# orottier/web-audio-api-rs

Measured on AMD Instinct MI355X. Metric: render quanta/sec (48kHz, 128-frame), higher is better.
Workload: dtype f64

## Files before the change

### web-audio-api-rs_amd/csrc/waa_biquad_lanes.hip

```cpp
#include <hip/hip_runtime.h>

#include <algorithm>
#include <cstdlib>
#include <type_traits>

#include "waa_internal.hpp"
#include "waa_stream_common.hpp"

namespace waa {

namespace {
struct V2 {
  double x, y;
};
struct M2 {
  double a, b, c, d;
};
__device__ __forceinline__ M2 mm(const M2& x, const M2& y) {
  M2 r;
  r.a = __builtin_fma(x.a, y.a, x.b * y.c);
  r.b = __builtin_fma(x.a, y.b, x.b * y.d);
  r.c = __builtin_fma(x.c, y.a, x.d * y.c);
  r.d = __builtin_fma(x.c, y.b, x.d * y.d);
  return r;
// ... 294 lines not shown
    for (int j = 0; j < 8; j++) {
      const int r = j * 8 + (lane >> 3);
      const uint32_t sr = g * 64u + (uint32_t)r;
      const bool r_live = sr < n_streams;
      const uint32_t ri = sr / (uint32_t)d.nch, rc = sr % (uint32_t)d.nch;
      orow[j] = r_live ? (uint32_t)((uint64_t)ri * d.out.inst_stride + (uint64_t)rc * d.out.ch_stride + f_tile + (uint64_t)(lane & 7) * 4)
                       : 0xFFFFFFFFu;
      if (FAST && d.debug == 1) orow[j] = (uint32_t)(((uint64_t)tile * n_groups + g) * 64 * TILE + r * CHUNK + (lane & 7) * 4);
    }
  }
  const uint64_t f_end = (uint64_t)d.n_quanta * RQ;
  const int n_chunk = f_tile + TILE <= f_end ? NCHUNK : (int)((f_end - f_tile + CHUNK - 1) / CHUNK);
  for (int c = 0; c < n_chunk; c++) {
    if (FAST || !slow_tile)
      stage_chunk(0, raw);
    else
      stage_chunk_slow(0, c);
    stage_tab(0);
    if (c + 1 < n_chunk) {
      if (FAST)
        fetch_chunk_fast(raw);
      else if (!slow_tile)
        fetch_chunk(c + 1, raw);
      fetch_tab((c + 1 + rot) & (NCHUNK - 1));
    }
    lds_sync();
    float* row = lds + lane * ROWF;
    const double* tb = tabs;
    if (d.debug == 3) {
    } else if (PASS == 0) {
#pragma unroll
      for (int k8 = 0; k8 < CHUNK / 8; k8++) {
        const f4v va = *reinterpret_cast<const f4v*>(row + k8 * 8), vb = *reinterpret_cast<const f4v*>(row + k8 * 8 + 4);
        const float xs[8] = {va.x, va.y, va.z, va.w, vb.x, vb.y, vb.z, vb.w};
#pragma unroll
        for (int e = 0; e < 8; e++) {
          const d2v h = *reinterpret_cast<const d2v*>(tb + 2 * (k8 * 8 + e));
          const double xd = (double)xs[e];
          z1 = __builtin_fma(h.x, xd, z1);
          z2 = __builtin_fma(h.y, xd, z2);
        }
        __builtin_amdgcn_sched_barrier(0);
      }
    } else {
#pragma unroll
      for (int k4 = 0; k4 < CHUNK / 4; k4++) {
        float yo[4];
        const f4v xv = *reinterpret_cast<const f4v*>(row + k4 * 4);
        const float x4[4] = {xv.x, xv.y, xv.z, xv.w};
#pragma unroll
        for (int h = 0; h < 2; h++) {
          double cs[10];
#pragma unroll
          for (int e = 0; e < 5; e++) {
            const d2v v = *reinterpret_cast<const d2v*>(tb + k4 * 20 + h * 10 + 2 * e);
            cs[2 * e] = v.x;
            cs[2 * e + 1] = v.y;
          }
#pragma unroll
          for (int e = 0; e < 2; e++) {
            const double b0 = cs[e * 5 + 0], b1 = cs[e * 5 + 1], b2 = cs[e * 5 + 2], a1 = cs[e * 5 + 3], a2 = cs[e * 5 + 4];
            const double xd = (double)x4[h * 2 + e];
            double y = (b0 * xd + b1 * x1) + b2 * x2;
            y = (y - a1 * y1) - a2 * y2;
            if (!__builtin_isfinite(y)) y = 0.;
            x2 = x1;
            x1 = xd;
            y2 = y1;
            y1 = y;
            float o = (float)y;
            if (d.n_gain > 0 && g0 != 1.f) o *= g0;
            if (d.n_gain > 1 && g1 != 1.f) o *= g1;
            yo[h * 2 + e] = mute ? 0.f : o;
          }
          __builtin_amdgcn_sched_barrier(0);
        }
        *reinterpret_cast<f4v*>(row + k4 * 4) = f4v{yo[0], yo[1], yo[2], yo[3]};
        __builtin_amdgcn_sched_barrier(0);
      }
    }
    lds_sync();
    if (PASS == 1) {
#pragma unroll
      for (int j = 0; j < 8; j++) {
        const int r = j * 8 + (lane >> 3);
        const f4v v = *reinterpret_cast<const f4v*>(lds + r * ROWF + (lane & 7) * 4);
        if (orow[j] != 0xFFFFFFFFu) {
          __builtin_nontemporal_store(v, (WAA_GLOBAL_AS f4v*)(d.out.base + orow[j]));
          orow[j] += FAST ? row_step : (uint32_t)CHUNK;
        }
      }
      lds_sync();
    }
  }
  if (PASS == 1) {
    for (int c = n_chunk; c < NCHUNK; c++) {
#pragma unroll
      for (int j = 0; j < 8; j++)
        if (orow[j] != 0xFFFFFFFFu) {
          __builtin_nontemporal_store(f4v{0.f, 0.f, 0.f, 0.f}, (WAA_GLOBAL_AS f4v*)(d.out.base + orow[j]));
          orow[j] += FAST ? row_step : (uint32_t)CHUNK;
        }
    }
  }
  if (!live) return;
  if (PASS == 0) {
    double* zp = d.z + ((uint64_t)tile * n_streams + sid) * 2;
    zp[0] = z1;
    zp[1] = z2;
  } else if (tile + 1 == d.tile1) {
    st[0] = x1;
    st[1] = x2;
    st[2] = y1;
    st[3] = y2;
  }
}

__global__ __launch_bounds__(256) void biquad_lanes_chain_kernel(const BiquadLanesDesc d) {
  const uint32_t n_streams = d.n_inst * (uint32_t)d.nch;
  const uint32_t sid = blockIdx.x * 256 + threadIdx.x;
  if (sid >= n_streams) return;
  const uint32_t inst = sid / (uint32_t)d.nch;
  const int ch = (int)(sid % (uint32_t)d.nch);
  const double* st = d.state + (uint64_t)inst * STATE_STRIDE + ch * 4;
  double s1 = st[2], s2 = st[3];
  for (uint32_t t0 = d.tile0; t0 < d.tile1; t0 += 8) {
    double zz[8][2];
#pragma unroll
    for (int k = 0; k < 8; k++) {
      const uint32_t t = t0 + k < d.tile1 ? t0 + k : d.tile1 - 1;
      const double* zp = d.z + ((uint64_t)t * n_streams + sid) * 2;
      zz[k][0] = load_global(zp);
      zz[k][1] = load_global(zp + 1);
    }
#pragma unroll
    for (int k = 0; k < 8; k++) {
      const uint32_t t = t0 + k;
      if (t >= d.tile1) break;
      double* sp = d.sin + ((uint64_t)t * n_streams + sid) * 2;
      sp[0] = s1;
      sp[1] = s2;
      const double* pt = d.ht + (uint64_t)t * BIQUAD_HT_WORDS + 2 * TILE + 4;
      const double n1 = __builtin_fma(pt[0], s1, __builtin_fma(pt[1], s2, zz[k][0]));
      const double n2 = __builtin_fma(pt[2], s1, __builtin_fma(pt[3], s2, zz[k][1]));
      s1 = n1;
      s2 = n2;
    }
  }
  double* xs = d.z + ((uint64_t)d.tile0 * n_streams + sid) * 2;
  xs[0] = st[0];
  xs[1] = st[1];
}

void launch_biquad_tile_digest(const BiquadLanesDesc& d, void* stream) {
  hipLaunchKernelGGL(biquad_tile_digest_kernel, dim3(d.n_tiles), dim3(64), 0, (hipStream_t)stream, d);
}
void launch_biquad_lanes(const BiquadLanesDesc& d0, void* stream) {
  BiquadLanesDesc d = d0;
  d.debug = measure_switch("WAA_LANES_DEBUG") ? (uint32_t)atoi(measure_switch("WAA_LANES_DEBUG")) : 0u;
  const uint32_t n_streams = d.n_inst * (uint32_t)d.nch, n_groups = (n_streams + 63u) / 64u;
  const size_t lds_a = 64 * ROWF * sizeof(float) + CHUNK * 2 * sizeof(double);
  const size_t lds_b = 64 * ROWF * sizeof(float) + CHUNK * 5 * sizeof(double);
  const uint32_t tf = measure_switch("WAA_LANES_GENERAL") ? d.tile0 : std::min(std::max(d.fast_tiles, d.tile0), d.tile1);
  auto pass = [&](auto pass_c) {
    constexpr int PASS = decltype(pass_c)::value;
    const size_t lds = (PASS == 0 ? lds_a : lds_b) + (measure_switch("WAA_LANES_LDS_PAD") ? (size_t)atoi(measure_switch("WAA_LANES_LDS_PAD")) : 0);
    if (tf > d.tile0) {
      d.lt0 = d.tile0;
      d.lt1 = tf;
      hipLaunchKernelGGL((biquad_lanes_kernel<PASS, true>), dim3((tf - d.tile0) * n_groups), dim3(64), lds, (hipStream_t)stream, d);
    }
    if (tf < d.tile1) {
      d.lt0 = tf;
      d.lt1 = d.tile1;
      hipLaunchKernelGGL((biquad_lanes_kernel<PASS, false>), dim3((d.tile1 - tf) * n_groups), dim3(64), lds, (hipStream_t)stream, d);
    }
  };
  pass(std::integral_constant<int, 0>{});
  hipLaunchKernelGGL(biquad_lanes_chain_kernel, dim3((n_streams + 255) / 256), dim3(256), 0, (hipStream_t)stream, d);
  pass(std::integral_constant<int, 1>{});
}

}
```

### web-audio-api-rs_amd/csrc/waa_internal.hpp

```cpp
#pragma once
#include <cstdint>
#include <cstdlib>

#include "waa_conv_noise.hpp"

namespace waa {

inline const char* measure_switch(const char* name) {
#ifdef WAA_MEASURE
  return getenv(name);
#else
  (void)name;
  return nullptr;
#endif
}

void raise_lds_limit(const void* kernel);

constexpr int RQ = 128;
constexpr int TILE_K = 32;
constexpr int TILE = 64 * TILE_K;
constexpr int QUANTA_PER_TILE = TILE / RQ;
constexpr int MAX_OPS = 12;
constexpr int MAX_INPUTS = 4;
// ... 4 lines not shown
  const float* base;
  uint64_t stride;
  int32_t mode;
  int32_t pad;
};

struct SignalRef {
  float* base;
  uint64_t inst_stride;
  uint64_t ch_stride;
  int32_t nch;
  int32_t pad;
};

enum : uint32_t { Q_SILENT = 0, Q_FAST = 1, Q_SLOW = 2, Q_FAST_LOOP = 3 };
struct QRec {
  int64_t start;
  uint32_t mode;
  uint32_t pad;
};
struct SlowRec {
  int32_t prev;
  int32_t next;
  double k;
};
struct SrcSchedule {
  const QRec* qrec;
  const SlowRec* slow;
  const uint8_t* tile_fast;
};
struct SrcInst {
  const float* base;
  uint64_t ch_stride;
  uint64_t frames;
  uint32_t sched;
  uint32_t aligned;
  SrcSchedule sc;
  int64_t linear_start;
  uint32_t fast_prefix;
  uint32_t linear_all;
};

enum : int32_t { IN_SILENT = 0, IN_SIGNAL = 1, IN_SOURCE = 2, IN_CONSTANT = 3, IN_DELAYED = 4 };
struct InputRef {
  int32_t kind;
  int32_t nch;
  SignalRef sig;
  const SrcInst* src;
  const SrcSchedule* sched;
  ParamRef offset;
  const int64_t* active;
  double sample_rate;
  int32_t num_quanta;
  int32_t feedback;
  uint64_t valid;
  ParamRef gain;
  int32_t has_gain;
  uint32_t fast_tiles;
  float delay_lo, delay_hi;
};

enum : int32_t {
  OP_GAIN = 1,
  OP_BIQUAD = 2,
  OP_WAVESHAPER = 3,
  OP_STEREO_PAN = 4,
  OP_PANNER = 5,
  OP_MIX = 6,
  OP_IIR = 7,
  OP_PARAM_ADD = 8
};
struct OpDesc {
  int32_t kind;
  int32_t nch_in;
  int32_t nch_out;
  int32_t i1;
  int32_t i2;
  int32_t i0;
  ParamRef p0;
  ParamRef p1;
  ParamRef p2;
  ParamRef p3;
  ParamRef p4;
  const void* ptr0;
  void* ptr1;
  const void* ptr2;
  uint64_t u0;
};

struct ChainDesc {
  int32_t n_inputs;
  int32_t in_nch;
  int32_t in_interp;
  int32_t n_ops;
  InputRef in[MAX_INPUTS];
  OpDesc ops[MAX_OPS];
  SignalRef out;
  uint32_t n_inst;
  uint32_t n_tiles;
  uint32_t n_quanta;
  uint32_t xcd_remap;
  uint32_t tile0, tile1;
  int32_t lds_curve_op;
  int32_t tile_major;
  uint32_t persist_block;
  uint32_t pad;
};

struct BiquadStreamDesc {
  InputRef in;
  const double* coefs;
  uint64_t coef_stride;
  int32_t vary;
  int32_t pad0;
  double* state;
  const double* hp;
  ParamRef gain[2];
  int32_t n_gain;
  int32_t nch;
  SignalRef out;
  uint32_t n_inst;
  uint32_t n_tiles;
  uint32_t n_quanta;
  uint32_t dup_out;
  uint32_t tile0, tile1;
};
void launch_biquad_stream(const BiquadStreamDesc& d, void* stream);
constexpr int BIQUAD_SCAN_PW = 88;
struct BiquadScanCtl {
  uint32_t* counter;
  uint32_t counter_base[8];
  double* payload;
  const double* pw;
  uint32_t* error;
};
void launch_biquad_scan_powers(const double* coefs, uint64_t coef_stride, double* pw, uint32_t n_inst, void* stream);
void launch_biquad_scan(const BiquadStreamDesc& d, const BiquadScanCtl& ctl, uint32_t* issued, void* stream);

constexpr int BIQUAD_HT_WORDS = 2 * TILE + 8;
struct BiquadLanesDesc {
  InputRef in;
  const double* coefs;
  double* ht;
  double* z;
  double* sin;
  double* state;
  ParamRef gain[2];
  int32_t n_gain, nch;
  SignalRef out;
  uint32_t n_inst, n_tiles, n_quanta, tile0, tile1;
  uint32_t fast_tiles;
  uint32_t lt0, lt1;
  uint32_t debug, pad;
};
void launch_biquad_tile_digest(const BiquadLanesDesc& d, void* stream);
void launch_biquad_lanes(const BiquadLanesDesc& d, void* stream);

struct IirStreamDesc {
  InputRef in;
  const double* coef;
  const double* pow;
  double* state;
  int32_t ns;
  int32_t nch;
  SignalRef out;
  uint32_t n_inst;
  uint32_t n_tiles;
  uint32_t n_quanta;
  uint32_t exact;
  uint32_t tile0, tile1;
  uint32_t coef_stride, pow_stride;
};
int iir_padded_states(int n_states);
void launch_iir_stream(const IirStreamDesc& d, void* stream);

struct CompRow {
  float thr, lo, hi, half_knee;
  float knee_partial, ratio, makeup, pad;
  float a_tau, a_one, r_tau, r_one;
};
struct CompDesc {
  SignalRef in;
  uint64_t in_valid;
  SignalRef out;
  float* xl;
  const CompRow* rows;
  uint32_t row_inst_stride, row_q_stride;
  uint32_t n_inst, n_quanta;
  uint64_t frames;
  uint32_t delay_frames;
  int32_t nch;
};
void launch_compressor_level(const CompDesc& d, void* stream);
void launch_compressor_detector(const CompDesc& d, void* stream);
void launch_compressor_apply(const CompDesc& d, void* stream);

enum : int32_t { RT_CHANNEL = 0, RT_DOWN2 = 1, RT_DOWN4 = 2, RT_DOWN6 = 3 };
struct RouteTerm {
  const float* base;
  uint64_t inst_stride, ch_stride;
  int32_t mode;
  int32_t ch;
};
struct RouteDesc {
  SignalRef out;
  const RouteTerm* terms;
  const uint32_t* row_off;
  uint32_t n_inst, rows;
  uint64_t frames;
};
void launch_route(const RouteDesc& d, void* stream);

struct ConvTerm {
  int32_t in_ch, ir_ch, out_ch, pad;
};
struct Cplx {
  float re, im;
};
struct ConvDesc {
  SignalRef in, out;
  int32_t n_terms;
  int32_t cin, cout;
  int32_t n;
  int32_t block;
  int32_t parts;
  int32_t nb;
  int32_t fft3;
  ConvTerm terms[4];
  const Cplx* H;
  Cplx* X;
  Cplx* Y;
  const Cplx* tw;
  const float* ir;
  uint64_t ir_len;
  uint64_t frames;
  uint64_t in_valid;
  uint32_t n_inst, n_pairs;
  int32_t ir_nch, pad1;
  int32_t kb0, kb1;
  int32_t mac_grid_order, pad2;
  const double* pre_coefs;
  uint64_t pre_coef_stride;
  double* pre_state;
  uint64_t ir_inst_stride;
  int32_t per_inst, pad3;
};
struct AnalyserDesc {
  SignalRef sig;
  uint32_t n_inst;
  int32_t fft_size;
  uint64_t frames_written;
  float smoothing;
  float min_db, max_db;
  int32_t pad;
  const float* window;
  const Cplx* tw;
  const Cplx* tw_full;
  const float* prev;
  float* db_out;
  uint8_t* byte_out;
  float* time_out;
  const uint8_t* code;
  uint64_t code_stride;
};
void launch_analyser(const AnalyserDesc& d, void* stream);
struct AnalyserSeriesDesc {
  AnalyserDesc a;
  int32_t first, hop;
  int32_t pulls;
  int32_t run;
  int32_t stage_span;
  int32_t lin;
  uint64_t frames;
  float* db_out;
  uint8_t* byte_out;
  float* time_out;
  uint8_t* tbyte_out;
};
void analyser_series_shape(AnalyserSeriesDesc* d);
void launch_analyser_series_fft(const AnalyserSeriesDesc& d, void* stream);
void launch_analyser_series_smooth(const AnalyserSeriesDesc& d, void* stream);
void launch_analyser_series_bytes(const AnalyserSeriesDesc& d, void* stream);
void launch_analyser_series_time(const AnalyserSeriesDesc& d, void* stream);
constexpr int DIRECT_MAX_TAPS = 128;
void launch_conv_direct(const ConvDesc& d, void* stream);
void launch_conv_ir_spectra(const ConvDesc& d, void* stream);
void launch_conv_forward(const ConvDesc& d, void* stream);
void launch_conv_mac(const ConvDesc& d, void* stream);
void launch_conv_inverse(const ConvDesc& d, void* stream);
void launch_conv3_ir_spectra(const ConvDesc& d, void* stream);
void launch_conv3_forward(const ConvDesc& d, void* stream);
void launch_conv3_inverse(const ConvDesc& d, void* stream);
void launch_conv_inst_direct(const ConvDesc& d, void* stream);
void launch_conv_inst_mac(const ConvDesc& d, void* stream);

struct DelayDesc {
  SignalRef in, out;
  ParamRef delay;
  double sample_rate;
  uint64_t frames;
  int32_t num_quanta;
  int32_t nch;
  uint32_t n_inst;
  uint32_t n_quanta;
  uint32_t tile0, tile1;
  int32_t in_cycle;
  int32_t pad;
  double quantum_duration;
};
// ... 434 lines not shown
```

### web-audio-api-rs_amd/csrc/waa_plan.cpp

```cpp
#include <array>
#include <set>

#include <memory>

#include "waa_host.hpp"
#include "waa_plan_parts.hpp"

namespace waa {
namespace host {

int prepare_source_input(waa_batch* b, uint32_t id, InputRef* in);
int validate_plan(waa_batch* b);

int device_timeline_param(waa_batch* b, const ParamStore& p, ParamRef* ref) {
  if (p.dev_ready) {
    *ref = p.dev_ref;
    return 0;
  }
  std::vector<TlHeader> hdr(b->n_inst);
  std::vector<TlEvent> events;
  std::vector<float> curves;
  for (uint32_t i = 0; i < b->n_inst; i++) {
    TlHeader& h = hdr[i];
    std::memset(&h, 0, sizeof h);
// ... 566 lines not shown
    bool serial = false;
    std::string desc;
    for (auto& o : ops) {
      serial |= o.kind == OP_BIQUAD;
      char t[64];
      if (o.kind == OP_MIX)
        snprintf(t, sizeof t, "MIX(%d->%d)", o.nch_in, o.nch_out);
      else if (o.kind == OP_BIQUAD)
        snprintf(t, sizeof t, "BIQUAD(%s)", o.i0 == 0 ? "const" : o.i0 == 1 ? "k-rate" : "a-rate");
      else
        snprintf(t, sizeof t, "%s", op_name(o.kind));
      desc += desc.empty() ? t : std::string(",") + t;
    }
    std::string ins;
    for (auto& in : inputs) {
      char t[48];
      snprintf(t, sizeof t, "%s%s:%dch", in.has_gain ? "gain*" : "", input_kind_name(in.kind), in.nch);
      ins += ins.empty() ? t : std::string("+") + t;
    }
    plan_note(b, "chain %s C=%d in=[%s]->%dch ops=[%s] out=%dch", serial ? "serial" : "parallel", cmax, ins.c_str(), in_nch,
              desc.c_str(), out.nch);
  }
  return 0;
}

int temp_signal(waa_batch* b, int nch, SignalRef* out) {
  float* p = nullptr;
  int e = dev_alloc(b, &p, (size_t)b->n_inst * nch * b->lp);
  if (e) return e;
  *out = SignalRef{p, (uint64_t)nch * b->lp, b->lp, nch, 0};
  return 0;
}

int emit_segments(waa_batch* b, std::vector<InputRef> inputs, int in_nch, int in_interp, const std::vector<OpDesc>& ops,
                  const SignalRef& out) {
  bool any_stream = false;
  const int max_mode = measure_switch("WAA_NO_KRATE_STREAM") ? 0 : (measure_switch("WAA_NO_ARATE_STREAM") ? 1 : 2);
  auto streams = [&](const OpDesc& o) { return o.kind == OP_IIR || (o.kind == OP_BIQUAD && o.i0 <= max_mode && o.nch_in <= MAX_CH); };
  for (auto& o : ops) any_stream |= streams(o);
  if (!any_stream) return push_chain_step(b, inputs, in_nch, in_interp, ops, out);
  std::vector<OpDesc> pending;
  int cur_nch = in_nch;
  size_t i = 0;
  while (i < ops.size()) {
    const OpDesc& o = ops[i];
    if (!streams(o)) {
      pending.push_back(o);
      cur_nch = o.nch_out;
      i++;
      continue;
    }
    const bool iir_exact = o.kind == OP_IIR && o.i0 < 0;
    const bool plain = pending.empty() && inputs.size() == 1 && !inputs[0].has_gain &&
                       ((inputs[0].kind == IN_SOURCE && !iir_exact) || (inputs[0].kind == IN_SIGNAL && inputs[0].valid == 0)) &&
                       inputs[0].nch == cur_nch;
    if (!plain) {
      SignalRef tmp;
      int e = temp_signal(b, cur_nch, &tmp);
      if (e) return e;
      if ((e = push_chain_step(b, inputs, in_nch, in_interp, pending, tmp))) return e;
      pending.clear();
      InputRef in{};
      in.kind = IN_SIGNAL;
      in.nch = cur_nch;
      in.sig = tmp;
      inputs.assign(1, in);
      in_nch = cur_nch;
    }
    size_t j = i + 1;
    if (o.kind == OP_BIQUAD)
      while (j < ops.size() && j - i <= 2 && ops[j].kind == OP_GAIN && ops[j].p0.mode == 0 && ops[j].nch_in == cur_nch) j++;
    const bool dup = o.kind == OP_BIQUAD && o.i0 == 0 && cur_nch == 1 && out.nch == 2 && j + 1 == ops.size() && ops[j].kind == OP_MIX &&
                     ops[j].nch_in == 1 && ops[j].nch_out == 2 && ops[j].i0 == WAA_INTERP_SPEAKERS && !measure_switch("WAA_NO_STREAM_DUP");
    SignalRef seg_out = out;
    if (!dup && (j < ops.size() || out.nch != cur_nch)) {
      int e = temp_signal(b, cur_nch, &seg_out);
      if (e) return e;
    }
    if (o.kind == OP_IIR) {
      Step st;
      st.kind = StepKind::IirStream;
      IirStreamDesc& q = st.iir;
      std::memset(&q, 0, sizeof q);
      q.in = inputs[0];
      q.coef = reinterpret_cast<const double*>(o.ptr0);
      q.pow = reinterpret_cast<const double*>(o.ptr2);
      q.state = reinterpret_cast<double*>(o.ptr1);
      q.ns = std::abs(o.i0);
      q.coef_stride = (uint32_t)o.u0;
      q.pow_stride = o.u0 && !iir_exact ? 6u * (uint32_t)(q.ns * q.ns) : 0u;
      q.exact = 0u;
      if (iir_exact) {
        const double streams = (double)b->n_inst * cur_nch;
        const double lane_cost = std::ceil(streams / 64. / 1024.) * (12. * q.ns + 32.);
        const double row_cost = std::ceil(streams / 4. / 1024.) * 64.;
        q.exact = (row_cost < lane_cost && !measure_switch("WAA_IIR_LANE")) || measure_switch("WAA_IIR_ROW") ? 2u : 1u;
      }
      q.nch = cur_nch;
      q.out = seg_out;
      q.n_inst = b->n_inst;
      q.n_tiles = b->n_tiles;
      q.tile0 = 0;
      q.tile1 = b->n_tiles;
      q.n_quanta = b->n_quanta;
      char name[40], per[40] = "";
      snprintf(name, sizeof name, "%s<%d%s>", q.exact == 2 ? "iir_row_kernel" : q.exact == 1 ? "iir_lane_kernel" : "iir_stream_kernel", q.ns,
               q.coef_stride ? ",inst" : "");
      st.profile_slot = slot_for(b, name);
      b->steps.push_back(st);
      if (q.coef_stride) snprintf(per, sizeof per, " coef=per-instance(%d)", o.i1);
      plan_note(b, "%s states=%d in=%s:%dch out=%s%s", q.exact == 2 ? "iir_exact(row)" : q.exact == 1 ? "iir_exact(lane)" : "iir_stream", q.ns,
                input_kind_name(inputs[0].kind), cur_nch, seg_out.base == out.base ? "final" : "temp", per);
      InputRef in{};
      in.kind = IN_SIGNAL;
      in.nch = cur_nch;
      in.sig = seg_out;
      inputs.assign(1, in);
      in_nch = cur_nch;
      i = j;
      if (i == ops.size() && seg_out.base == out.base) return 0;
      continue;
    }
    if (o.kind == OP_BIQUAD && o.i0 == 2 && !dup && b->steps[(size_t)o.i1].coef.rows == 1 && !measure_switch("WAA_ARATE_STREAM") &&
        (inputs[0].kind == IN_SIGNAL || inputs[0].kind == IN_SOURCE) &&
        (uint64_t)b->n_inst * seg_out.inst_stride < (1ull << 32)) {
      Step& cstep = b->steps[(size_t)o.i1];
      Step& dstep = b->steps[(size_t)o.i1 + 1];
      cstep.coef.lane_major = 0;
      const size_t n_streams = (size_t)b->n_inst * cur_nch;
      double *ht = nullptr, *z = nullptr, *sin = nullptr;
      int e;
      if ((e = dev_alloc(b, &ht, (size_t)b->n_tiles * BIQUAD_HT_WORDS)) || (e = dev_alloc(b, &z, (size_t)b->n_tiles * n_streams * 2)) ||
          (e = dev_alloc(b, &sin, (size_t)b->n_tiles * n_streams * 2)))
        return e;
      BiquadLanesDesc L;
      std::memset(&L, 0, sizeof L);
      L.in = inputs[0];
      L.coefs = cstep.coef.coefs;
      L.ht = ht;
      L.z = z;
      L.sin = sin;
      L.state = reinterpret_cast<double*>(o.ptr1);
      L.n_gain = (int)(j - i - 1);
      for (size_t k = i + 1; k < j; k++) L.gain[k - i - 1] = ops[k].p0;
      L.nch = cur_nch;
      L.out = seg_out;
      L.n_inst = b->n_inst;
      L.n_tiles = b->n_tiles;
      L.n_quanta = b->n_quanta;
      L.tile0 = 0;
      L.tile1 = b->n_tiles;
      L.fast_tiles = inputs[0].kind == IN_SOURCE ? inputs[0].fast_tiles
                                                 : (inputs[0].valid ? (uint32_t)std::min<uint64_t>(inputs[0].valid / TILE, b->n_tiles) : b->n_tiles);
      dstep.kind = StepKind::BiquadTileDigest;
      dstep.lanes = L;
      dstep.profile_slot = slot_for(b, "biquad_tile_digest_kernel");
      Step ls;
      ls.kind = StepKind::BiquadLanes;
      ls.lanes = L;
      ls.profile_slot = slot_for(b, "biquad_lanes_kernel");
      b->steps.push_back(ls);
      plan_note(b, "biquad_lanes(a-rate, shared table: one lane per stream, tiles in parallel) in=%s:%dch gains=%d out=%s",
                input_kind_name(inputs[0].kind), cur_nch, L.n_gain, seg_out.base == out.base ? "final" : "temp");
      InputRef in{};
      in.kind = IN_SIGNAL;
      in.nch = cur_nch;
      in.sig = seg_out;
      inputs.assign(1, in);
      in_nch = cur_nch;
      i = j;
      if (i == ops.size() && seg_out.base == out.base) return 0;
      continue;
    }
    Step st;
    st.kind = StepKind::BiquadStream;
    BiquadStreamDesc& q = st.bq;
    std::memset(&q, 0, sizeof q);
    q.in = inputs[0];
    q.coefs = reinterpret_cast<const double*>(o.ptr0);
    q.coef_stride = o.u0;
    q.vary = o.i0;
    if (o.i0 == 2) {
      Step& cstep = b->steps[(size_t)o.i1];
      cstep.coef.lane_major = 1;
      if (cstep.coef.rows == 1 && !measure_switch("WAA_NO_ARATE_DIGEST")) {
        Step& hstep = b->steps[(size_t)o.i1 + 1];
        double* dhp = nullptr;
        int e = dev_alloc(b, &dhp, (size_t)b->n_tiles * HP_WORDS * 64);
        if (e) return e;
        hstep.hp.coefs = cstep.coef.coefs;
        hstep.hp.hp = dhp;
        hstep.hp.n_tiles = b->n_tiles;
        q.hp = dhp;
        q.vary = 3;
      }
    }
    q.state = reinterpret_cast<double*>(o.ptr1);
    q.n_gain = (int)(j - i - 1);
    for (size_t k = i + 1; k < j; k++) q.gain[k - i - 1] = ops[k].p0;
    q.nch = cur_nch;
    q.out = seg_out;
    q.dup_out = dup ? 1u : 0u;
    q.n_inst = b->n_inst;
    q.n_tiles = b->n_tiles;
    q.tile0 = 0;
    q.tile1 = b->n_tiles;
    q.n_quanta = b->n_quanta;
    st.profile_slot = slot_for(b, "biquad_stream_kernel");
    if (q.vary == 0 && !b->dry && measure_switch("WAA_BIQUAD_SCAN")) {
      const size_t n_streams = (size_t)b->n_inst * cur_nch;
      if (!b->scan_counter) {
        int e = dev_alloc(b, &b->scan_counter, 8 * 16 + 16);
        if (e) return e;
        b->state_bufs.push_back({b->scan_counter, (8 * 16 + 16) * sizeof(uint32_t)});
      }
      double *payload = nullptr, *pw = nullptr;
      int e;
      if ((e = dev_alloc(b, &payload, n_streams * b->n_tiles * 8)) || (e = dev_alloc(b, &pw, (size_t)b->n_inst * BIQUAD_SCAN_PW)))
        return e;
      b->ones_bufs.push_back({payload, n_streams * b->n_tiles * 8 * sizeof(double)});
      launch_biquad_scan_powers(q.coefs, q.coef_stride, pw, b->n_inst, b->stream);
      HIP_TRY(hipGetLastError());
      st.scan.counter = b->scan_counter;
      st.scan.error = b->scan_counter + 8 * 16;
      st.scan.payload = payload;
      st.scan.pw = pw;
      st.profile_slot = slot_for(b, "biquad_scan_kernel");
    }
    b->steps.push_back(st);
    if (dup) {
      plan_note(b, "biquad_stream in=%s:1ch gains=%d out=final (both channels: the speakers up-mix 1 -> 2 behind it)",
                input_kind_name(inputs[0].kind), q.n_gain);
      return 0;
    }
    plan_note(b, "biquad_stream%s in=%s:%dch gains=%d out=%s",
              q.vary == 3 ? "(a-rate, shared table)" : q.vary == 2 ? "(a-rate, per-instance table)" : q.vary ? "(k-rate)" : "",
              input_kind_name(inputs[0].kind),
              cur_nch, q.n_gain, seg_out.base == out.base ? "final" : "temp");
    InputRef in{};
    in.kind = IN_SIGNAL;
    in.nch = cur_nch;
    in.sig = seg_out;
    inputs.assign(1, in);
    in_nch = cur_nch;
    i = j;
    if (i == ops.size() && seg_out.base == out.base) return 0;
  }
  return push_chain_step(b, inputs, in_nch, in_interp, pending, out);
}

bool is_delay(const waa_batch* b, uint32_t id) { return b->nodes[id].desc.kind == WAA_NODE_DELAY; }
void vertex_targets(const waa_batch* b, uint32_t v, const std::vector<uint8_t>& cut, std::vector<uint32_t>& out) {
  const uint32_t id = v & ~VTX_READER;
  if (!(v & VTX_READER) && is_delay(b, id)) {
    if (!cut[id]) out.push_back(id | VTX_READER);
    return;
  }
  for (auto& e : b->edges) {
    if (e.from != id) continue;
    out.push_back(is_delay(b, e.to) && (e.to_input & 0x80000000u) ? (e.to | VTX_READER) : e.to);
  }
}

int materialise_automation(waa_batch* b) {
  const double sample_rate = (double)b->sr, dt = 1. / sample_rate;
  for (Node& n : b->nodes)
    for (size_t pk = 0; pk < n.params.size(); pk++) {
      ParamStore& p = n.params[pk];
      if (p.timelines.empty()) continue;
      bool shared = p.timelines_shared && p.timelines[0];
      for (uint32_t i = 1; i < b->n_inst && shared; i++) shared = p.cst[i] == p.cst[0] && p.timelines[i];
      {
        const uint32_t kind = n.desc.kind;
        const bool consumable = kind == WAA_NODE_GAIN || kind == WAA_NODE_BIQUAD || kind == WAA_NODE_DELAY ||
                                kind == WAA_NODE_STEREO_PANNER || kind == WAA_NODE_CONSTANT_SOURCE ||
                                kind == WAA_NODE_OSCILLATOR ||
                                (kind == WAA_NODE_PANNER && pk >= 6 && n.desc.i[0] != WAA_PANNING_HRTF);
        const bool want = measure_switch("WAA_DEVICE_AUTOMATION") ? true : !shared;
        bool arrivals = false;
        for (const auto& tl : p.timelines) arrivals |= tl && tl->has_arrivals();
        if (consumable && !p.k_rate && want && !arrivals && !b->dry && !measure_switch("WAA_HOST_AUTOMATION")) {
          p.dev_tl = true;
          continue;
        }
      }
      for (uint32_t inst = 0; inst < (shared ? 1u : b->n_inst); inst++) {
        Timeline* tl = p.timelines[inst].get();
        if (!tl) continue;
        float buf[RQ];
        ParamBlock run;
        run.inst = shared ? WAA_ALL_INSTANCES : inst;
        run.nq = 0;
        auto flush = [&] {
          if (run.nq) p.blocks.push_back(run);
          run.nq = 0;
          run.v.clear();
        };
        for (uint32_t q = 0; q < b->n_quanta; q++) {
          const double block_time = (double)((uint64_t)q * RQ) / sample_rate;
          if (int ea = tl->apply_arrivals(q)) return ea;
          const uint32_t len = tl->compute(block_time, dt, RQ, buf);
          if (run.nq && run.vpq != len) flush();
          if (!run.nq) {
            run.q0 = q;
            run.vpq = len;
          }
// ... 1284 lines not shown
```

### web-audio-api-rs_amd/csrc/waa_plan_check.cpp

```cpp
#include <array>
#include <set>

#include "waa_host.hpp"
#include "waa_plan_parts.hpp"

namespace waa {
namespace host {

void io_param(const ParamRef& p, StepIo& io) {
  if (p.base && p.mode == 2) io.reads.push_back(p.base);
}
void io_input(const InputRef& in, StepIo& io) {
  if (in.kind == IN_SIGNAL || (in.kind == IN_DELAYED && !in.feedback)) io.reads.push_back(in.sig.base);
  if (in.kind == IN_CONSTANT) io_param(in.offset, io);
  if (in.has_gain) io_param(in.gain, io);
}
static StepIo step_io_raw(const Step& st);
StepIo step_io(const waa_batch* b, const Step& st) {
  StepIo io = step_io_raw(st);
  if (!b->view_owner.empty())
    for (const void*& r : io.reads) {
      auto it = b->view_owner.find(r);
      if (it != b->view_owner.end()) r = it->second;
    }
  return io;
}
static StepIo step_io_raw(const Step& st) {
  StepIo io;
  switch (st.kind) {
    case StepKind::Chain: {
      const ChainDesc& c = st.chain;
      for (int k = 0; k < c.n_inputs; k++) io_input(c.in[k], io);
      for (int o = 0; o < c.n_ops; o++) {
        const OpDesc& op = c.ops[o];
        io_param(op.p0, io);
        io_param(op.p1, io);
        io_param(op.p2, io);
        io_param(op.p3, io);
        io_param(op.p4, io);
        if (op.kind == OP_BIQUAD && op.i0 == 2) io.reads.push_back(op.ptr0);
      }
      io.writes.push_back(c.out.base);
      break;
    }
    case StepKind::BiquadStream:
      io_input(st.bq.in, io);
      if (st.bq.vary >= 2) io.reads.push_back(st.bq.coefs);
      if (st.bq.vary == 3) io.reads.push_back(st.bq.hp);
      io.writes.push_back(st.bq.out.base);
      break;
    case StepKind::ConvFft:
    case StepKind::ConvDirect:
      io.reads.push_back(st.conv.in.base);
      io.writes.push_back(st.conv.out.base);
      break;
    case StepKind::Compressor:
      io.reads.push_back(st.comp.in.base);
      io.writes.push_back(st.comp.out.base);
      break;
    case StepKind::ZeroFill:
      io.writes.push_back(st.zero_ptr);
      break;
    case StepKind::BiquadCoefs:
      io_param(st.coef.frequency, io);
      io_param(st.coef.detune, io);
      io_param(st.coef.q, io);
      io_param(st.coef.gain, io);
      io.writes.push_back(st.coef.coefs);
      break;
    case StepKind::Timeline:
      io.writes.push_back(st.tl.out);
      break;
    case StepKind::PannerGeom:
      for (int k = 0; k < 15; k++) io_param(st.geom.p[k], io);
      io.writes.push_back(st.geom.az);
      io.writes.push_back(st.geom.gl_mono);
      io.writes.push_back(st.geom.gr_mono);
      io.writes.push_back(st.geom.gl_stereo);
      io.writes.push_back(st.geom.gr_stereo);
      io.writes.push_back(st.geom.dg);
      io.writes.push_back(st.geom.cg);
      break;
    case StepKind::BiquadHp:
      if (st.hp.coefs) {
        io.reads.push_back(st.hp.coefs);
        io.writes.push_back(st.hp.hp);
      }
      break;
    case StepKind::BiquadTileDigest:
      io.reads.push_back(st.lanes.coefs);
      io.writes.push_back(st.lanes.ht);
      break;
    case StepKind::BiquadLanes:
      io_input(st.lanes.in, io);
      io.reads.push_back(st.lanes.coefs);
      io.reads.push_back(st.lanes.ht);
      io.writes.push_back(st.lanes.out.base);
      break;
    case StepKind::IirStream:
      io_input(st.iir.in, io);
      io.writes.push_back(st.iir.out.base);
      break;
    case StepKind::Delay:
      io.reads.push_back(st.delay.in.base);
      io_param(st.delay.delay, io);
      io.writes.push_back(st.delay.out.base);
      io.feedback_reader = st.delay.in_cycle != 0;
      break;
    case StepKind::Route:
    case StepKind::Loop:
    case StepKind::Dyn:
    case StepKind::QGemm:
    case StepKind::Hrtf:
    case StepKind::OsFft:
      io.reads = st.loop_reads;
      io.writes = st.loop_writes;
      break;
    case StepKind::Osc:
      io_param(st.osc.frequency, io);
      io_param(st.osc.detune, io);
      io.writes.push_back(st.osc.out.base);
      break;
    case StepKind::ConvCodes:
    case StepKind::Link:
      break;
  }
  return io;
}

int validate_plan(waa_batch* b) {
  std::vector<StepIo> ios;
  std::set<const void*> produced, written;
  for (const Step& st : b->steps) {
    ios.push_back(step_io(b, st));
    for (const void* w : ios.back().writes)
      if (w) produced.insert(w);
  }
  for (size_t k = 0; k < b->steps.size(); k++) {
    const StepIo& io = ios[k];
    const StepKind kind = b->steps[k].kind;
    if (kind == StepKind::Loop || kind == StepKind::Dyn) {
      for (const void* w : io.writes) written.insert(w);
    }
    for (const void* r : io.reads) {
      if (!r || !produced.count(r) || written.count(r)) continue;
      if (io.feedback_reader && r == b->steps[k].delay.in.base) continue;
      return fail(WAA_ERR_INVALID_STATE, "internal: launch %zu of the plan (kind %d, %s) reads a buffer that a later launch produces", k,
                  (int)kind, step_traits(kind).name);
    }
    for (const void* w : io.writes)
      if (w) written.insert(w);
  }
  return 0;
}

}
}
```

Before: 2.916 billion.

## Add single-pass biquad lanes kernel with decoupled look-back across blocks

Adds a one-pass biquad path for the fast tiles. A new piece-digest kernel precomputes per-piece impulse responses and 2x2 state-transition matrices. A new lanes kernel then lets each workgroup compute its local block response, publish it, and chain the incoming state from predecessor blocks via a decoupled look-back with anchors, spinning on status flags, before running the exact recursion and writing output. This is meant to replace the previous two-pass scheme and cut the extra passes over the input. In exchange it adds several device buffers, cross-workgroup spin-waits that rely on ticket ordering for forward progress, and an error flag for timeouts.

New measurement: 2.941 billion, median of 4. Within noise of the previous version (+0.9%).

```diff
diff --git a/web-audio-api-rs_amd/csrc/waa_biquad_lanes.hip b/web-audio-api-rs_amd/csrc/waa_biquad_lanes.hip
--- a/web-audio-api-rs_amd/csrc/waa_biquad_lanes.hip
+++ b/web-audio-api-rs_amd/csrc/waa_biquad_lanes.hip
@@ -470,11 +470,24 @@
   xs[1] = st[1];
 }
 
+static bool lanes_one_pass(const BiquadLanesDesc& d) {
+  return d.rec && d.fast_tiles > 0 && !measure_switch("WAA_LANES_TWO_PASS") && !measure_switch("WAA_LANES_GENERAL");
+}
 void launch_biquad_tile_digest(const BiquadLanesDesc& d, void* stream) {
-  hipLaunchKernelGGL(biquad_tile_digest_kernel, dim3(d.n_tiles), dim3(64), 0, (hipStream_t)stream, d);
+  const bool one_pass = lanes_one_pass(d);
+  if (one_pass) launch_biquad_piece_digest(d, stream);
+  if (!one_pass || d.fast_tiles < d.n_tiles)
+    hipLaunchKernelGGL(biquad_tile_digest_kernel, dim3(d.n_tiles), dim3(64), 0, (hipStream_t)stream, d);
 }
 void launch_biquad_lanes(const BiquadLanesDesc& d0, void* stream) {
   BiquadLanesDesc d = d0;
+  if (lanes_one_pass(d) && d.tile0 < std::min(d.fast_tiles, d.tile1)) {
+    d.lt0 = d.tile0;
+    d.lt1 = std::min(d.fast_tiles, d.tile1);
+    launch_biquad_lanes1(d, stream);
+    if (d.lt1 == d.tile1) return;
+    d.tile0 = d.lt1;
+  }
   d.debug = measure_switch("WAA_LANES_DEBUG") ? (uint32_t)atoi(measure_switch("WAA_LANES_DEBUG")) : 0u;
   const uint32_t n_streams = d.n_inst * (uint32_t)d.nch, n_groups = (n_streams + 63u) / 64u;
   const size_t lds_a = 64 * ROWF * sizeof(float) + CHUNK * 2 * sizeof(double);
diff --git a/web-audio-api-rs_amd/csrc/waa_biquad_lanes1.hip b/web-audio-api-rs_amd/csrc/waa_biquad_lanes1.hip
--- /dev/null
+++ b/web-audio-api-rs_amd/csrc/waa_biquad_lanes1.hip
@@ -0,0 +1,427 @@
+#include <hip/hip_runtime.h>
+
+#include <atomic>
+
+#include "waa_internal.hpp"
+#include "waa_stream_common.hpp"
+
+namespace waa {
+
+namespace {
+struct V2 {
+  double x, y;
+};
+struct M2 {
+  double a, b, c, d;
+};
+__device__ __forceinline__ M2 mm(const M2& x, const M2& y) {
+  M2 r;
+  r.a = __builtin_fma(x.a, y.a, x.b * y.c);
+  r.b = __builtin_fma(x.a, y.b, x.b * y.d);
+  r.c = __builtin_fma(x.c, y.a, x.d * y.c);
+  r.d = __builtin_fma(x.c, y.b, x.d * y.d);
+  return r;
+}
+__device__ __forceinline__ V2 mvv(const M2& m, const V2& v) { return V2{__builtin_fma(m.a, v.x, m.b * v.y), __builtin_fma(m.c, v.x, m.d * v.y)}; }
+constexpr int F = LANES1_F;
+constexpr int W = LANES1_W;
+constexpr int BLOCK = LANES1_BLOCK;
+constexpr int BPT = TILE / BLOCK;
+constexpr int PTW = LANES1_PT_WORDS;
+constexpr int CHUNK = 32;
+constexpr int ROWS = 64 * CHUNK;
+constexpr int TABW = CHUNK * 5;
+constexpr uint32_t ANCHOR = 16;
+constexpr uint32_t SPIN_MAX = 1u << 18;
+constexpr size_t LDS_BYTES = (size_t)W * (ROWS * sizeof(float) + TABW * sizeof(double)) + 16 + 64 * sizeof(uint32_t);
+typedef const __attribute__((address_space(4))) double* cdp;
+typedef double d2v __attribute__((ext_vector_type(2)));
+__device__ __forceinline__ double ald(const double* p) { return __hip_atomic_load(p, __ATOMIC_RELAXED, __HIP_MEMORY_SCOPE_AGENT); }
+__device__ __forceinline__ void ast(double* p, double v) { __hip_atomic_store(p, v, __ATOMIC_RELAXED, __HIP_MEMORY_SCOPE_AGENT); }
+__device__ __forceinline__ uint32_t aldu(const uint32_t* p) { return __hip_atomic_load(p, __ATOMIC_RELAXED, __HIP_MEMORY_SCOPE_AGENT); }
+__device__ __forceinline__ void astu(uint32_t* p, uint32_t v) { __hip_atomic_store(p, v, __ATOMIC_RELAXED, __HIP_MEMORY_SCOPE_AGENT); }
+__device__ __forceinline__ void lds_barrier() { asm volatile("s_waitcnt lgkmcnt(0)\n\ts_barrier" ::: "memory"); }
+__device__ __forceinline__ int sw(int r, int c) { return r * CHUNK + ((c ^ ((r >> 1) & 7)) << 2); }
+}
+
+__global__ __launch_bounds__(64) void biquad_piece_digest_kernel(const BiquadLanesDesc d) {
+  __shared__ double sh[64][4];
+  const int lane = threadIdx.x;
+  const uint32_t n_pieces = d.n_tiles * (uint32_t)(TILE / F);
+  const uint32_t piece = blockIdx.x * 64u + (uint32_t)lane;
+  double pa = 1., pb = 0., pc = 0., pd = 1.;
+  if (piece < n_pieces) {
+    const cdp ct = (cdp)(d.coefs + (uint64_t)piece * F * 5);
+    double* out = d.pt + (uint64_t)piece * PTW;
+    double g1a = 0., g1c = 0., g2a = 0., g2c = 0.;
+    double b1n = 0., b2n = 0., b2nn = 0.;
+#pragma unroll 8
+    for (int i = F - 1; i >= 0; i--) {
+      const double b0 = ct[i * 5 + 0], b1 = ct[i * 5 + 1], b2 = ct[i * 5 + 2], a1 = ct[i * 5 + 3], a2 = ct[i * 5 + 4];
+      const double ga = pa + pb, gc = pc + pd;
+      out[2 * i] = ga * b0 + g1a * b1n + g2a * b2nn;
+      out[2 * i + 1] = gc * b0 + g1c * b1n + g2c * b2nn;
+      if (i == 0) {
+        out[2 * F + 0] = ga * b1 + g1a * b2n;
+        out[2 * F + 1] = gc * b1 + g1c * b2n;
+        out[2 * F + 2] = ga * b2;
+        out[2 * F + 3] = gc * b2;
+      }
+      g2a = g1a;
+      g2c = g1c;
+      g1a = ga;
+      g1c = gc;
+      b2nn = b2n;
+      b1n = b1;
+      b2n = b2;
+      const double pp = -a1 - a2;
+      const double na = pa * pp + pb * (pp - 1.), nc = pc * pp + pd * (pp - 1.);
+      pb = ga * a2;
+      pd = gc * a2;
+      pa = na;
+      pc = nc;
+    }
+    out[2 * F + 4] = pa;
+    out[2 * F + 5] = pb;
+    out[2 * F + 6] = pc;
+    out[2 * F + 7] = pd;
+  }
+  sh[lane][0] = pa;
+  sh[lane][1] = pb;
+  sh[lane][2] = pc;
+  sh[lane][3] = pd;
+  __syncthreads();
+  const uint32_t block = blockIdx.x * (64u / W) + (uint32_t)lane;
+  if (lane < 64 / W && block < d.n_tiles * (uint32_t)BPT) {
+    M2 Q = {1., 0., 0., 1.};
+    for (int v = 0; v < W; v++) {
+      double* q = d.pt + ((uint64_t)block * W + v) * PTW + 2 * F + 8;
+      q[0] = Q.a;
+      q[1] = Q.b;
+      q[2] = Q.c;
+      q[3] = Q.d;
+      Q = mm(M2{sh[lane * W + v][0], sh[lane * W + v][1], sh[lane * W + v][2], sh[lane * W + v][3]}, Q);
+    }
+    double* o = d.pb + (uint64_t)block * 4;
+    o[0] = Q.a;
+    o[1] = Q.b;
+    o[2] = Q.c;
+    o[3] = Q.d;
+  }
+}
+
+__global__ __launch_bounds__(64 * W, 4) void biquad_lanes1_kernel(const BiquadLanesDesc d) {
+  extern __shared__ __attribute__((aligned(16))) float lds[];
+  const int lane = threadIdx.x & 63;
+  const int w = __builtin_amdgcn_readfirstlane((int)(threadIdx.x >> 6));
+  float* rows = lds + w * ROWS;
+  double* tab = reinterpret_cast<double*>(lds + W * ROWS) + w * TABW;
+  uint32_t* ctl = reinterpret_cast<uint32_t*>(reinterpret_cast<double*>(lds + W * ROWS) + W * TABW);
+  uint32_t* obase = ctl + 4;
+  __builtin_amdgcn_s_setreg(1 | (6 << 6) | (1 << 11), 0);
+  auto lds_sync = []() __attribute__((always_inline)) { __builtin_amdgcn_wave_barrier(); };
+  const uint32_t n_streams = d.n_inst * (uint32_t)d.nch;
+  const uint32_t n_groups = (n_streams + 63u) / 64u;
+  const uint32_t b_first = d.tile0 * (uint32_t)BPT, n_blk = (d.lt1 - d.tile0) * (uint32_t)BPT, n_blk_all = d.n_tiles * (uint32_t)BPT;
+  const uint32_t n_units = n_blk * n_groups;
+  if (threadIdx.x == 0) ctl[0] = __hip_atomic_fetch_add(d.ctl, 1u, __ATOMIC_RELAXED, __HIP_MEMORY_SCOPE_AGENT);
+  lds_barrier();
+  const uint32_t ticket = (uint32_t)__builtin_amdgcn_readfirstlane((int)ctl[0]);
+  if (ticket >= n_units) {
+    if (threadIdx.x == 0) astu(d.error, 1u);
+    return;
+  }
+  const uint32_t rb = ticket / n_groups, blk = b_first + rb, g = ticket % n_groups;
+  const bool anchor = rb % ANCHOR == 0u;
+  const uint32_t sid = g * 64u + (uint32_t)lane;
+  const bool live = sid < n_streams;
+  const uint32_t inst = live ? sid / (uint32_t)d.nch : 0u;
+  const int ch = live ? (int)(sid % (uint32_t)d.nch) : 0;
+  const float* base;
+  if (d.in.kind == IN_SOURCE) {
+    const SrcInst* sp = d.in.src + inst;
+    base = load_global(&sp->base) + (uint64_t)ch * load_global(&sp->ch_stride) + load_global(&sp->linear_start);
+  } else {
+    base = d.in.sig.base + (uint64_t)inst * d.in.sig.inst_stride + (uint64_t)ch * d.in.sig.ch_stride;
+  }
+  double* st = d.state + (uint64_t)inst * STATE_STRIDE + ch * 4;
+  const uint64_t f_blk = (uint64_t)blk * BLOCK, f_piece = f_blk + (uint64_t)(w * F);
+  const uint64_t f_end = (uint64_t)d.n_quanta * RQ;
+  const bool piece_live = f_piece < f_end;
+  f4v raw[16];
+#pragma unroll
+  for (int j = 0; j < 8; j++) {
+    const int r = j * 8 + (lane >> 3);
+    const bool r_live = g * 64u + (uint32_t)r < n_streams;
+    const uint64_t pb = (uint64_t)__shfl((unsigned long long)(uintptr_t)base, r_live ? r : 0, 64);
+    const float* p = reinterpret_cast<const float*>(pb) + f_piece + (uint64_t)(lane & 7) * 4;
+    if (piece_live) {
+      raw[j] = __builtin_nontemporal_load((const WAA_GLOBAL_AS f4v*)p);
+      raw[8 + j] = __builtin_nontemporal_load((const WAA_GLOBAL_AS f4v*)(p + CHUNK));
+    } else {
+      raw[j] = raw[8 + j] = f4v{0.f, 0.f, 0.f, 0.f};
+    }
+  }
+  d2v xh = {0., 0.};
+  if (w == 0 && live && piece_live) {
+    if (blk == b_first) {
+      xh.x = st[0];
+      xh.y = st[1];
+    } else {
+      xh.x = (double)load_global(base + f_blk - 1);
+      xh.y = (double)load_global(base + f_blk - 2);
+    }
+  }
+  const d2v hraw = *(const WAA_GLOBAL_AS d2v*)(d.pt + (uint64_t)(blk * W + (uint32_t)w) * PTW + 2 * lane);
+  const double* tsrc = d.coefs + f_piece * 5;
+  d2v traw[2];
+  auto fetch_tab = [&](int c) __attribute__((always_inline)) {
+    const double* p = tsrc + c * TABW;
+    traw[0] = *(const WAA_GLOBAL_AS d2v*)(p + 2 * lane);
+    traw[1] = *(const WAA_GLOBAL_AS d2v*)(p + 128 + (lane < 16 ? 2 * lane : 0));
+  };
+  auto stage_tab = [&]() __attribute__((always_inline)) {
+    *reinterpret_cast<d2v*>(tab + 2 * lane) = traw[0];
+    if (lane < 16) *reinterpret_cast<d2v*>(tab + 128 + 2 * lane) = traw[1];
+  };
+  float x[F];
+#pragma unroll
+  for (int c = 0; c < 2; c++) {
+#pragma unroll
+    for (int j = 0; j < 8; j++) *reinterpret_cast<f4v*>(rows + sw(j * 8 + (lane >> 3), lane & 7)) = raw[c * 8 + j];
+    if (c == 0) *reinterpret_cast<d2v*>(tab + 2 * lane) = hraw;
+    lds_sync();
+#pragma unroll
+    for (int k = 0; k < 8; k++) {
+      const f4v v = *reinterpret_cast<const f4v*>(rows + sw(lane, k));
+      x[c * CHUNK + k * 4 + 0] = v.x;
+      x[c * CHUNK + k * 4 + 1] = v.y;
+      x[c * CHUNK + k * 4 + 2] = v.z;
+      x[c * CHUNK + k * 4 + 3] = v.w;
+    }
+    lds_sync();
+  }
+  double z1 = 0., z2 = 0.;
+#pragma unroll
+  for (int k8 = 0; k8 < F / 8; k8++) {
+#pragma unroll
+    for (int e = 0; e < 8; e++) {
+      const d2v h = *reinterpret_cast<const d2v*>(tab + 2 * (k8 * 8 + e));
+      float xf = x[k8 * 8 + e];
+      asm volatile("" : "+v"(xf));
+      const double xd = (double)xf;
+      z1 = __builtin_fma(h.x, xd, z1);
+      z2 = __builtin_fma(h.y, xd, z2);
+    }
+    __builtin_amdgcn_sched_barrier(0);
+  }
+  {
+    char* ex = reinterpret_cast<char*>(rows) + lane * 48;
+    *reinterpret_cast<d2v*>(ex) = d2v{z1, z2};
+    float xl1 = x[F - 1], xl2 = x[F - 2];
+    asm volatile("" : "+v"(xl1), "+v"(xl2));
+    *reinterpret_cast<d2v*>(ex + 16) = d2v{(double)xl1, (double)xl2};
+    if (w == 0) {
+      *reinterpret_cast<d2v*>(ex + 32) = xh;
+      obase[lane] = live ? (uint32_t)((uint64_t)inst * d.out.inst_stride + (uint64_t)ch * d.out.ch_stride) : 0xFFFFFFFFu;
+    }
+  }
+  lds_barrier();
+  V2 Y = {0., 0.}, Yw = {0., 0.}, xin = {0., 0.};
+  {
+    const cdp pt0 = (cdp)(d.pt + (uint64_t)blk * W * PTW);
+    const d2v xh0 = *reinterpret_cast<const d2v*>(reinterpret_cast<const char*>(lds) + lane * 48 + 32);
+    V2 xp = {xh0.x, xh0.y};
+#pragma unroll
+    for (int v = 0; v < W; v++) {
+      const char* exv = reinterpret_cast<const char*>(lds + v * ROWS) + lane * 48;
+      if (v == w) {
+        Yw = Y;
+        xin = xp;
+      }
+      const d2v zv = *reinterpret_cast<const d2v*>(exv), xl = *reinterpret_cast<const d2v*>(exv + 16);
+      const cdp t = pt0 + v * PTW + 2 * F;
+      const M2 P = {t[4], t[5], t[6], t[7]};
+      const double e1 = zv.x + __builtin_fma(t[0], xp.x, t[2] * xp.y), e2 = zv.y + __builtin_fma(t[1], xp.x, t[3] * xp.y);
+      const V2 py = mvv(P, Y);
+      Y = V2{py.x + e1, py.y + e2};
+      xp = V2{xl.x, xl.y};
+    }
+  }
+  fetch_tab(0);
+  const uint32_t seq = d.seq;
+  double* recp = d.rec + ((uint64_t)blk * n_groups + g) * LANES1_REC_WORDS;
+  uint32_t* statp = d.stat + (uint64_t)g * n_blk_all + blk;
+  if (w == 0) {
+    uint32_t n = 0;
+    if (rb != 0u) {
+      if (!anchor) {
+        ast(recp + 2 * lane, Y.x);
+        ast(recp + 2 * lane + 1, Y.y);
+        asm volatile("s_waitcnt vmcnt(0)" ::: "memory");
+        if (lane == 0) astu(statp, seq * 4u + 1u);
+      }
+      const uint32_t want = rb - (rb - 1u) / ANCHOR * ANCHOR;
+      const unsigned long long all = (1ull << want) - 1ull;
+      uint32_t spins = 0;
+      for (;;) {
+        uint32_t s = 0;
+        if ((uint32_t)lane < want) {
+          const uint32_t v = aldu(statp - 1 - lane);
+          s = (v >> 2) == seq ? (v & 3u) : 0u;
+        }
+        if ((__ballot((uint32_t)lane + 1u == want ? s == 2u : s >= 1u) & all) == all) {
+          n = want;
+          break;
+        }
+        __builtin_amdgcn_s_sleep(1);
+        if (++spins > SPIN_MAX) {
+          if (lane == 0) astu(d.error, 1u);
+          break;
+        }
+      }
+    }
+    if (lane == 0) ctl[1] = n;
+  }
+  lds_barrier();
+  const uint32_t n = (uint32_t)__builtin_amdgcn_readfirstlane((int)ctl[1]);
+  V2 part = {0., 0.};
+  if (n > 0) {
+    M2 M = {1., 0., 0., 1.};
+    for (uint32_t k = 0; k < n; k++) {
+      const uint32_t j = blk - 1u - k;
+      if ((k & (uint32_t)(W - 1)) == (uint32_t)w) {
+        const double* rp = d.rec + ((uint64_t)j * n_groups + g) * LANES1_REC_WORDS + (k == n - 1u ? 128 : 0) + 2 * lane;
+        const V2 t = mvv(M, V2{ald(rp), ald(rp + 1)});
+        part.x += t.x;
+        part.y += t.y;
+      }
+      const cdp pj = (cdp)(d.pb + (uint64_t)j * 4);
+      M = mm(M, M2{pj[0], pj[1], pj[2], pj[3]});
+    }
+  } else if (w == 0 && rb == 0u && live) {
+    part.x = st[2];
+    part.y = st[2] - st[3];
+  }
+  *reinterpret_cast<d2v*>(reinterpret_cast<char*>(rows) + 4096 + lane * 16) = d2v{part.x, part.y};
+  lds_barrier();
+  V2 S = {0., 0.};
+#pragma unroll
+  for (int v = 0; v < W; v++) {
+    const d2v p = *reinterpret_cast<const d2v*>(reinterpret_cast<const char*>(lds + v * ROWS) + 4096 + lane * 16);
+    S.x += p.x;
+    S.y += p.y;
+  }
+  lds_barrier();
+  if (w == 0 && anchor) {
+    const cdp pq = (cdp)(d.pb + (uint64_t)blk * 4);
+    const V2 ps = mvv(M2{pq[0], pq[1], pq[2], pq[3]}, S);
+    ast(recp + 128 + 2 * lane, ps.x + Y.x);
+    ast(recp + 128 + 2 * lane + 1, ps.y + Y.y);
+    asm volatile("s_waitcnt vmcnt(0)" ::: "memory");
+    if (lane == 0) astu(statp, seq * 4u + 2u);
+  }
+  int ls = lane;
+  asm volatile("" : "+v"(ls));
+  const uint32_t ocol = (uint32_t)f_piece + (uint32_t)(ls & 7) * 4u;
+  if (!piece_live) {
+#pragma unroll
+    for (int c = 0; c < 2; c++)
+#pragma unroll
+      for (int j = 0; j < 8; j++)
+      {
+        const uint32_t ob = obase[j * 8 + (ls >> 3)];
+        if (ob != 0xFFFFFFFFu) __builtin_nontemporal_store(f4v{0.f, 0.f, 0.f, 0.f}, (WAA_GLOBAL_AS f4v*)(d.out.base + (ob + ocol + c * CHUNK)));
+      }
+  } else {
+    float g0 = 1.f, g1 = 1.f;
+    bool mute = false;
+    if (live) {
+      if (d.n_gain > 0) g0 = d.gain[0].base[inst];
+      if (d.n_gain > 1) g1 = d.gain[1].base[inst];
+      mute = (d.n_gain > 0 && fabsf(g0) <= 1e-6f) || (d.n_gain > 1 && fabsf(g1) <= 1e-6f);
+      if (fabsf(1.f - g0) <= 1e-6f) g0 = 1.f;
+      if (fabsf(1.f - g1) <= 1e-6f) g1 = 1.f;
+    }
+    const cdp qw = (cdp)(d.pt + (uint64_t)(blk * W + (uint32_t)w) * PTW + 2 * F + 8);
+    const V2 s0 = mvv(M2{qw[0], qw[1], qw[2], qw[3]}, S);
+    double y1 = s0.x + Yw.x, y2 = y1 - (s0.y + Yw.y), x1 = xin.x, x2 = xin.y;
+#pragma unroll
+    for (int c = 0; c < 2; c++) {
+      stage_tab();
+      if (c == 0) fetch_tab(1);
+      lds_sync();
+#pragma unroll
+      for (int k4 = 0; k4 < CHUNK / 4; k4++) {
+        float yo[4];
+#pragma unroll
+        for (int h = 0; h < 2; h++) {
+          double cs[10];
+#pragma unroll
+          for (int e = 0; e < 5; e++) {
+            const d2v v = *reinterpret_cast<const d2v*>(tab + k4 * 20 + h * 10 + 2 * e);
+            cs[2 * e] = v.x;
+            cs[2 * e + 1] = v.y;
+          }
+#pragma unroll
+          for (int e = 0; e < 2; e++) {
+            const double b0 = cs[e * 5 + 0], b1 = cs[e * 5 + 1], b2 = cs[e * 5 + 2], a1 = cs[e * 5 + 3], a2 = cs[e * 5 + 4];
+            const double xd = (double)x[c * CHUNK + k4 * 4 + h * 2 + e];
+            double y = (b0 * xd + b1 * x1) + b2 * x2;
+            y = (y - a1 * y1) - a2 * y2;
+            if (!__builtin_isfinite(y)) y = 0.;
+            x2 = x1;
+            x1 = xd;
+            y2 = y1;
+            y1 = y;
+            float o = (float)y;
+            if (d.n_gain > 0 && g0 != 1.f) o *= g0;
+            if (d.n_gain > 1 && g1 != 1.f) o *= g1;
+            yo[h * 2 + e] = mute ? 0.f : o;
+          }
+          __builtin_amdgcn_sched_barrier(0);
+        }
+        *reinterpret_cast<f4v*>(rows + sw(lane, k4)) = f4v{yo[0], yo[1], yo[2], yo[3]};
+        __builtin_amdgcn_sched_barrier(0);
+      }
+      lds_sync();
+#pragma unroll
+      for (int j = 0; j < 8; j++) {
+        const f4v v = *reinterpret_cast<const f4v*>(rows + sw(j * 8 + (ls >> 3), ls & 7));
+        const uint32_t ob = obase[j * 8 + (ls >> 3)];
+        if (ob != 0xFFFFFFFFu) __builtin_nontemporal_store(v, (WAA_GLOBAL_AS f4v*)(d.out.base + (ob + ocol + c * CHUNK)));
+      }
+      lds_sync();
+    }
+    const uint64_t f_last = (uint64_t)d.lt1 * TILE < f_end ? (uint64_t)d.lt1 * TILE : f_end;
+    if (live && f_piece + F == f_last) {
+      st[0] = x1;
+      st[1] = x2;
+      st[2] = y1;
+      st[3] = y2;
+    }
+  }
+  if (threadIdx.x == 0) {
+    const uint32_t done = __hip_atomic_fetch_add(d.ctl + 1, 1u, __ATOMIC_RELAXED, __HIP_MEMORY_SCOPE_AGENT);
+    if (done + 1u == n_units) {
+      astu(d.ctl, 0u);
+      astu(d.ctl + 1, 0u);
+    }
+  }
+}
+
+void launch_biquad_piece_digest(const BiquadLanesDesc& d, void* stream) {
+  const uint32_t n_pieces = d.n_tiles * (uint32_t)(TILE / F);
+  hipLaunchKernelGGL(biquad_piece_digest_kernel, dim3((n_pieces + 63) / 64), dim3(64), 0, (hipStream_t)stream, d);
+}
+
+void launch_biquad_lanes1(const BiquadLanesDesc& d0, void* stream) {
+  static std::atomic<uint32_t> launches{0};
+  BiquadLanesDesc d = d0;
+  d.seq = launches.fetch_add(1u) % 0x3FFFFFF0u + 1u;
+  const uint32_t n_streams = d.n_inst * (uint32_t)d.nch, n_groups = (n_streams + 63u) / 64u;
+  raise_lds_limit(reinterpret_cast<const void*>(biquad_lanes1_kernel));
+  hipLaunchKernelGGL(biquad_lanes1_kernel, dim3((d.lt1 - d.tile0) * (uint32_t)BPT * n_groups), dim3(64 * W), LDS_BYTES, (hipStream_t)stream, d);
+}
+
+}
diff --git a/web-audio-api-rs_amd/csrc/waa_internal.hpp b/web-audio-api-rs_amd/csrc/waa_internal.hpp
--- a/web-audio-api-rs_amd/csrc/waa_internal.hpp
+++ b/web-audio-api-rs_amd/csrc/waa_internal.hpp
@@ -180,9 +180,23 @@
   uint32_t fast_tiles;
   uint32_t lt0, lt1;
   uint32_t debug, pad;
-};
+  double* pt;
+  double* pb;
+  double* rec;
+  uint32_t* stat;
+  uint32_t* ctl;
+  uint32_t* error;
+  uint32_t seq, pad1;
+};
+constexpr int LANES1_F = 64;
+constexpr int LANES1_W = 8;
+constexpr int LANES1_BLOCK = LANES1_F * LANES1_W;
+constexpr int LANES1_PT_WORDS = 2 * LANES1_F + 12;
+constexpr int LANES1_REC_WORDS = 256;
 void launch_biquad_tile_digest(const BiquadLanesDesc& d, void* stream);
 void launch_biquad_lanes(const BiquadLanesDesc& d, void* stream);
+void launch_biquad_piece_digest(const BiquadLanesDesc& d, void* stream);
+void launch_biquad_lanes1(const BiquadLanesDesc& d, void* stream);
 
 struct IirStreamDesc {
   InputRef in;
diff --git a/web-audio-api-rs_amd/csrc/waa_plan.cpp b/web-audio-api-rs_amd/csrc/waa_plan.cpp
--- a/web-audio-api-rs_amd/csrc/waa_plan.cpp
+++ b/web-audio-api-rs_amd/csrc/waa_plan.cpp
@@ -742,6 +742,18 @@
       L.tile1 = b->n_tiles;
       L.fast_tiles = inputs[0].kind == IN_SOURCE ? inputs[0].fast_tiles
                                                  : (inputs[0].valid ? (uint32_t)std::min<uint64_t>(inputs[0].valid / TILE, b->n_tiles) : b->n_tiles);
+      if (!b->dry && L.fast_tiles > 0) {
+        const size_t n_blocks = (size_t)b->n_tiles * (TILE / LANES1_BLOCK), n_groups = (n_streams + 63) / 64;
+        if (!b->scan_counter) {
+          if ((e = dev_alloc(b, &b->scan_counter, 8 * 16 + 16))) return e;
+          b->state_bufs.push_back({b->scan_counter, (8 * 16 + 16) * sizeof(uint32_t)});
+        }
+        if ((e = dev_alloc(b, &L.pt, (size_t)b->n_tiles * (TILE / LANES1_F) * LANES1_PT_WORDS)) || (e = dev_alloc(b, &L.pb, n_blocks * 4)) ||
+            (e = dev_alloc(b, &L.rec, n_blocks * n_groups * LANES1_REC_WORDS)) || (e = dev_alloc(b, &L.stat, n_groups * n_blocks)))
+          return e;
+        L.error = b->scan_counter + 8 * 16;
+        L.ctl = b->scan_counter + 8 * 16 + 8;
+      }
       dstep.kind = StepKind::BiquadTileDigest;
       dstep.lanes = L;
       dstep.profile_slot = slot_for(b, "biquad_tile_digest_kernel");
diff --git a/web-audio-api-rs_amd/csrc/waa_plan_check.cpp b/web-audio-api-rs_amd/csrc/waa_plan_check.cpp
--- a/web-audio-api-rs_amd/csrc/waa_plan_check.cpp
+++ b/web-audio-api-rs_amd/csrc/waa_plan_check.cpp
@@ -90,11 +90,21 @@
     case StepKind::BiquadTileDigest:
       io.reads.push_back(st.lanes.coefs);
       io.writes.push_back(st.lanes.ht);
+      if (st.lanes.rec) {
+        io.writes.push_back(st.lanes.pt);
+        io.writes.push_back(st.lanes.pb);
+      }
       break;
     case StepKind::BiquadLanes:
       io_input(st.lanes.in, io);
       io.reads.push_back(st.lanes.coefs);
       io.reads.push_back(st.lanes.ht);
+      if (st.lanes.rec) {
+        io.reads.push_back(st.lanes.pt);
+        io.reads.push_back(st.lanes.pb);
+        io.writes.push_back(st.lanes.rec);
+        io.writes.push_back(st.lanes.stat);
+      }
       io.writes.push_back(st.lanes.out.base);
       break;
     case StepKind::IirStream:
```
